# rohithr87/CILRS-Autonomous-Driving-CARLA

Hardware: AMD Instinct MI355X
Metric: frames/sec CILRS train batch=128 (higher is better)
Workload: dtype f32; 1 GPU; CILRS ResNet-34 train step (fwd+loss+bwd+Adam), Config A, 200x88 RGB, B=128/GPU, fp32; global_batch=128, parallelism=single

## Files before the change

### cilrs-autonomous-driving-carla_amd/cilrs_mi355/_lib.py

```python
from __future__ import annotations

import ctypes as C
import os

_HERE = os.path.dirname(os.path.abspath(__file__))
LIB_PATH = os.environ.get("CILRS_LIB") or os.path.join(_HERE, "libcilrs_hip.so")

c_float_p = C.POINTER(C.c_float)
vp = C.c_void_p
sz = C.c_size_t
i32 = C.c_int
i64 = C.c_int64
f32 = C.c_float
f64 = C.c_double
u64 = C.c_uint64


class Buffers(C.Structure):
    _fields_ = [("params", vp), ("grads", vp), ("bn_running", vp), ("bn_nbt", vp),
                ("workspace", vp)]


class AdamArgs(C.Structure):
    _fields_ = [("exp_avg", vp), ("exp_avg_sq", vp), ("lr", C.c_double), ("beta1", C.c_double),
# ... 134 lines not shown
    "cilrs_augment_weather_u8": (i32, [vp, vp, vp, i32, i32, i32, vp, vp, vp]),
    "cilrs_batch_assemble_weather": (i32, [vp, i64, vp, vp, vp, vp, vp, vp, i32, i32, i32, vp, vp, vp,
                                           vp, vp, vp]),
    "cilrs_augment_view_u8": (i32, [vp, vp, vp, vp, i32, i32, i32, vp, vp, vp]),
    "cilrs_batch_assemble_view": (i32, [vp, i64, vp, vp, vp, vp, vp, vp, vp, i32, i32, i32, vp, vp,
                                        vp, vp, vp, vp]),
    "cilrs_eval_acc_doubles": (i32, []),
    "cilrs_eval_accumulate": (i32, [vp, vp, vp, vp, vp, i32, vp, vp, vp]),
    "cilrs_net_profile_enable": (i32, [vp, i32]),
    "cilrs_net_profile_collect": (i32, [vp]),
    "cilrs_net_profile_count": (i32, [vp]),
    "cilrs_net_profile_entry": (i32, [vp, i32, C.c_char_p, i32, C.POINTER(C.c_longlong),
                                      C.POINTER(f64), C.POINTER(f64), C.POINTER(f64)]),
    "cilrs_net_profile_reset": (i32, [vp]),
    "cilrs_conv2d_fwd": (i32, [vp, vp, vp] + [i32] * 11 + [vp, sz, vp]),
    "cilrs_conv2d_dgrad": (i32, [vp, vp, vp, vp] + [i32] * 11 + [vp, sz, vp]),
    "cilrs_conv2d_fwd_stats": (i32, [vp, vp, vp, vp, C.POINTER(i32)] + [i32] * 10 + [vp, sz, vp]),
    "cilrs_conv2d_dgrad_bnbwd": (i32, [vp] * 7 + [i32, vp, C.POINTER(i32)] + [i32] * 10
                                 + [vp, sz, vp]),
    "cilrs_conv2d_takes_classes": (i32, [i32] * 9 + [sz, i32]),
    "cilrs_net_conv_classes": (i32, [vp, i32, C.POINTER(i32), C.POINTER(i32)]),
    "cilrs_conv2d_wgrad_scratch_floats": (sz, [i32] * 9),
    "cilrs_conv2d_wgrad": (i32, [vp, vp, vp, vp] + [i32] * 10 + [vp]),
    "cilrs_conv2d_16_scratch_halfs": (sz, [i32] * 8),
    "cilrs_conv2d_fwd_16": (i32, [vp, vp, vp, vp] + [i32] * 9 + [vp, vp]),
    "cilrs_conv2d_dgrad_16": (i32, [vp, vp, vp, vp] + [i32] * 9 + [vp, vp]),
    "cilrs_conv2d_wgrad_16_scratch_floats": (sz, [i32] * 8),
    "cilrs_conv2d_wgrad_16": (i32, [vp, vp, vp, vp] + [i32] * 9 + [vp, vp]),
    "cilrs_conv2d_train_16": (i32, [vp] * 9 + [i32, vp] + [i32] * 12 + [vp, vp]),
    "cilrs_conv2d_infer_16": (i32, [vp] * 5 + [i32] * 11 + [vp]),
    "cilrs_stem_fold_16": (i32, [vp, vp, vp, vp, i32, vp]),
    "cilrs_stem_infer_16": (i32, [vp, vp, vp, vp, i32, i32, i32, i32, vp]),
    "cilrs_maxpool_infer_16": (i32, [vp, vp, i32, i32, i32, i32, i32, vp]),
    "cilrs_avgpool_infer_16": (i32, [vp, vp, i32, i32, i32, i32, i32, vp]),
    "cilrs_bn16_train_fwd": (i32, [vp, i32, i32, vp, vp, vp, vp, vp, C.c_float, C.c_float, vp, i32,
                                   vp, vp, vp, i32, vp]),
    "cilrs_bn16_bwd": (i32, [vp, vp, vp, i32, i32, vp, vp, i32, vp, vp, vp, vp, vp, vp, i32, vp]),
    "cilrs_conv2d_wino_split": (i32, [vp, vp, vp, vp, vp, i32, i32, i32, i32, i32, vp, sz, vp, vp, vp]),
    "cilrs_conv2d_wino_scratch_floats": (sz, [i32, i32]),
    "cilrs_conv2d_wino_fwd": (i32, [vp, vp, vp, i32, i32, i32, i32, i32, vp, vp]),
    "cilrs_conv2d_wino_fold_fwd": (i32, [vp, vp, vp, vp, vp, vp, i32, i32, i32, i32, i32, i32, i32,
                                         vp, vp]),
    "cilrs_wino_filter_transform": (i32, [vp, vp, i32, i32, i32, vp]),
    "cilrs_conv2d_wino_stamps": (i32, [vp]),
    "cilrs_conv2d_wino_pre": (i32, [vp, vp, vp, vp, i32, i32, i32, i32, i32, vp]),
    "cilrs_conv2d_wino_dgrad": (i32, [vp, vp, vp, vp, i32, i32, i32, i32, i32, vp, vp]),
# ... 60 lines not shown
```

### cilrs-autonomous-driving-carla_amd/csrc/common.h

```cpp
#pragma once
#include <hip/hip_runtime.h>
#include <stdint.h>
#include <stddef.h>
#include "../../include/cilrs_hip.h"

namespace cilrs {

typedef float f32x4 __attribute__((ext_vector_type(4)));
typedef float f32x16 __attribute__((ext_vector_type(16)));

void set_error(const char* fmt, ...);
const char* last_error();

#define CILRS_CHECK(cond, ...)                   \
    do {                                         \
        if (!(cond)) {                           \
            ::cilrs::set_error(__VA_ARGS__);     \
            return 1;                            \
        }                                        \
    } while (0)

#define CILRS_HIP(expr)                                                                 \
    do {                                                                                \
        hipError_t e_ = (expr);                                                         \
// ... 108 lines not shown
    if (mode < 16) return;
    const int units = mode - 16;
    const int k = (int)((blockIdx.x >> 8) % 5u);
    for (int i = 0; i < k * units; ++i) __builtin_amdgcn_s_sleep(1);
}
#endif
int wave_priority_mode();

struct WgradArgs {
    const float* x;
    const float* dy;
    float* dw;
    float* slabs;
    int N, H, W, Cin;
    int Ho, Wo, Cout;
    int KH, KW, stride, pad;
    int x_ld, dy_ld;
    int Cin_dst;
    int accumulate;
    int prio_mode;
};
size_t wgrad_scratch_floats(const WgradArgs& a);
int launch_conv_wgrad(const WgradArgs& a, hipStream_t s);

size_t bn_partial_floats(int C);
int launch_bn_train_fwd(const float* y, int M, int C, const float* gamma, const float* beta,
                        float* running_mean, float* running_var, long long* nbt, float momentum,
                        float eps, const float* residual, int relu, float* stats, float* partial,
                        float* z, int pre_nblk, hipStream_t s, void* z16 = nullptr,
                        double* acc_head = nullptr, double* acc = nullptr);
constexpr int kBnStatsHead = 2, kBnStatsRows = 4;
int launch_bn_train_stats(const float* y, int M, int C, double* acc, float* partial, hipStream_t s);
constexpr int kMaxConvs = 56;
struct BnEvalTable {
    int n;
    int C[kMaxConvs];
    unsigned gamma[kMaxConvs], beta[kMaxConvs];
    unsigned rm[kMaxConvs], rv[kMaxConvs];
    unsigned stats[kMaxConvs];
};
int launch_bn_eval_stats_all(const BnEvalTable& t, const float* params, const float* bn_running,
                             float* ws, float eps, hipStream_t s);
struct BnStatsTable {
    int n;
    int C[kMaxConvs];
    unsigned rm[kMaxConvs], rv[kMaxConvs];
// ... 499 lines not shown
```

### cilrs-autonomous-driving-carla_amd/csrc/conv_wgrad.hip

```cpp
#include "common.h"

#include <stdlib.h>

namespace cilrs {

namespace {

constexpr int BKP = 32;

template <int BT, bool TAP_UNIFORM, bool PIN>
__global__ __launch_bounds__(256, 2) void conv_wgrad_kernel(const WgradArgs a, const int Mpix,
                                                            const int splits, const int tiles_ci,
                                                            const int Ncols, const int ntiles_x,
                                                            const int ntiles_co,
                                                            const int xcd_group) {
    constexpr int WT = BT / 2, T = WT / 32;
    constexpr int QPR = BT / 4;
    constexpr int RPP = 256 / QPR;
    constexpr int PASSES = BKP / RPP;
    constexpr int PITCH = BT + 4;

    extern __shared__ __attribute__((aligned(16))) float smem[];
    float* As = smem;
    float* Bs = smem + 2 * BKP * PITCH;

    const int tid = threadIdx.x, lane = tid & 63, wave = tid >> 6;
    const int l31 = lane & 31, lh = lane >> 5;
    const int wm = wave >> 1, wn = wave & 1;
    wave_priority(a.prio_mode < 16 ? a.prio_mode : 0);

    int logical = (int)blockIdx.x;
    if (xcd_group) {
        const int nwg = (int)gridDim.x, bid = (int)blockIdx.x;
        const int q = nwg >> 3, r = nwg & 7, xcd = bid & 7;
        const int base = xcd < r ? xcd * (q + 1) : r * (q + 1) + (xcd - r) * q;
        logical = base + (bid >> 3);
    }
    const int ntile = logical % ntiles_x;
    const int co0 = ((logical / ntiles_x) % ntiles_co) * BT;
    const int z = logical / (ntiles_x * ntiles_co);

    const int KT = (Mpix + BKP - 1) / BKP;
    const int per = (KT + splits - 1) / splits;
    const int kt_begin = z * per;
    const int kt_end = min(KT, kt_begin + per);
    const int nt = max(kt_end - kt_begin, 0);

    const int q = tid % QPR, rr = tid / QPR;

    int tap, ci, col0;
    bool col_ok;
    if constexpr (TAP_UNIFORM) {
        tap = ntile / tiles_ci;
        ci = (ntile - tap * tiles_ci) * BT + q * 4;
        col0 = tap * a.Cin + (ntile - tap * tiles_ci) * BT;
        col_ok = true;
    } else {
        col0 = ntile * BT;
        const int j = col0 + q * 4;
        tap = j / a.Cin;
        ci = j - tap * a.Cin;
        col_ok = j < Ncols;
    }
    const int kh = tap / a.KW, kw = tap - kh * a.KW;
    const int HoWo = a.Ho * a.Wo;

    const int dn = BKP / HoWo, drem = BKP - dn * HoWo;
    const int doh = drem / a.Wo, dow = drem - doh * a.Wo;
    int cn[PASSES], coh[PASSES], cow[PASSES], cp[PASSES];
#pragma unroll
    for (int i = 0; i < PASSES; ++i) {
        const int p = kt_begin * BKP + rr + RPP * i;
        cp[i] = p;
        cn[i] = p / HoWo;
        const int rem = p - cn[i] * HoWo;
        coh[i] = rem / a.Wo;
        cow[i] = rem - coh[i] * a.Wo;
    }
    const __amdgpu_buffer_rsrc_t rsDy = __builtin_amdgcn_make_buffer_rsrc(
        (void*)a.dy, 0, (int)(unsigned)((size_t)Mpix * a.dy_ld * sizeof(float)), 0x00020000);
    const __amdgpu_buffer_rsrc_t rsX = __builtin_amdgcn_make_buffer_rsrc(
        (void*)a.x, 0, (int)(unsigned)((size_t)a.N * a.H * a.W * a.x_ld * sizeof(float)),
        0x00020000);
    const unsigned dyq = (unsigned)(co0 + q * 4) * 4u;
    const unsigned dy_pitch = (unsigned)a.dy_ld * 4u;

    auto load_tile = [&](f32x4(&ra)[PASSES], f32x4(&rb)[PASSES]) {
#pragma unroll
        for (int i = 0; i < PASSES; ++i) {
            const int h = coh[i] * a.stride - a.pad + kh, w = cow[i] * a.stride - a.pad + kw;
            const bool ok = col_ok && cp[i] < Mpix && h >= 0 && w >= 0 && h < a.H && w < a.W;
            const unsigned xo =
                ok ? (unsigned)(((cn[i] * a.H + h) * a.W + w) * a.x_ld + ci) * 4u : 0xFFFFFFFFu;
            ra[i] = __builtin_bit_cast(
                f32x4, __builtin_amdgcn_raw_buffer_load_b128(
                           rsDy, (int)((unsigned)cp[i] * dy_pitch + dyq), 0, 0));
            rb[i] = __builtin_bit_cast(
                f32x4, __builtin_amdgcn_raw_buffer_load_b128(rsX, (int)xo, 0, 0));
            cp[i] += BKP;
            cow[i] += dow;
            int c1 = cow[i] >= a.Wo;
            cow[i] -= c1 ? a.Wo : 0;
            coh[i] += doh + c1;
            int c2 = coh[i] >= a.Ho;
            coh[i] -= c2 ? a.Ho : 0;
            cn[i] += dn + c2;
        }
    };
    auto store_tile = [&](int buf, const f32x4(&ra)[PASSES], const f32x4(&rb)[PASSES]) {
#pragma unroll
        for (int i = 0; i < PASSES; ++i) {
            const int row = rr + RPP * i;
            *reinterpret_cast<f32x4*>(As + (buf * BKP + row) * PITCH + q * 4) = ra[i];
            *reinterpret_cast<f32x4*>(Bs + (buf * BKP + row) * PITCH + q * 4) = rb[i];
        }
    };

    f32x16 acc[T][T];
#pragma unroll
    for (int i = 0; i < T; ++i)
#pragma unroll
        for (int j = 0; j < T; ++j)
#pragma unroll
            for (int r = 0; r < 16; ++r) acc[i][j][r] = 0.f;

    auto compute = [&](int buf) {
        if constexpr (T == 2) {
            const float* Ab = As + buf * BKP * PITCH + lh * PITCH + wm * WT + 2 * l31;
// ... 76 lines not shown
        const int col = col0 + wn * WT + 2 * l31;
#pragma unroll
        for (int i = 0; i < 2; ++i)
#pragma unroll
            for (int r = 0; r < 16; ++r) {
                const int row = (r & 3) + 8 * (r >> 2) + 4 * lh;
                const int co = co0 + wm * WT + 2 * row + i;
                float2 v;
                v.x = acc[i][0][r];
                v.y = acc[i][1][r];
                *reinterpret_cast<float2*>(out + (size_t)co * Ncols + col) = v;
            }
    } else {
        const int col = col0 + wn * WT + l31;
#pragma unroll
        for (int r = 0; r < 16; ++r) {
            const int row = (r & 3) + 8 * (r >> 2) + 4 * lh;
            const int co = co0 + wm * WT + row;
            if (col < Ncols) out[(size_t)co * Ncols + col] = acc[0][0][r];
        }
    }
}

template <int VEC>
__global__ __launch_bounds__(256) void wgrad_reduce_kernel(const float* __restrict__ slabs,
                                                           float* __restrict__ dw,
                                                           const int splits, const size_t n_src,
                                                           const int cin, const int cin_dst,
                                                           const int accumulate, const int G) {
    if constexpr (VEC == 4) {
        __shared__ f32x4 red[256];
        const int opb = 256 / G;
        const int g = threadIdx.x / opb, ol = threadIdx.x - g * opb;
        const size_t nvec = n_src / 4;
        const size_t iv = (size_t)blockIdx.x * opb + ol;
        f32x4 v = {0.f, 0.f, 0.f, 0.f};
        if (iv < nvec) {
            const float* base = slabs + iv * 4;
            f32x4 acc[4];
#pragma unroll
            for (int u = 0; u < 4; ++u) acc[u] = f32x4{0.f, 0.f, 0.f, 0.f};
            int sidx = g;
            for (; sidx + 3 * G < splits; sidx += 4 * G) {
#pragma unroll
                for (int u = 0; u < 4; ++u)
                    acc[u] += *reinterpret_cast<const f32x4*>(base + (size_t)(sidx + u * G) * n_src);
// ... 27 lines not shown
#pragma unroll
                for (int u = 0; u < 4; ++u) acc[u] += base[(size_t)(sidx + u * G) * n_src];
            }
            for (; sidx < splits; sidx += G) acc[0] += base[(size_t)sidx * n_src];
            v = (acc[0] + acc[1]) + (acc[2] + acc[3]);
        }
        if (G > 1) {
            red1[threadIdx.x] = v;
            __syncthreads();
            if (g == 0) {
                for (int k = 1; k < G; ++k) v += red1[k * opb + ol];
            }
        }
        if (g == 0 && idx < n_src) {
            const int ci = (int)(idx % cin);
            if (ci < cin_dst) {
                const size_t o = (idx / cin) * cin_dst + ci;
                dw[o] = accumulate ? dw[o] + v : v;
            }
        }
    }
}

struct WPlan { int bt; bool uniform; int tiles_ci; int ntiles; int ncols; int splits; };

double wplan_cost(double flops, int tiles, int splits, int bt, size_t out_floats) {
    static const float r128[2] = {105.f, 120.f};
    static const float r64[4] = {60.f, 85.f, 96.f, 103.f};
    const int occ = bt == 128 ? 2 : 4;
    const float* rate = bt == 128 ? r128 : r64;
    const long blocks = (long)tiles * splits;
    const long per_cu = (blocks + 255) / 256;
    const double unit = flops / (double)blocks;
    const long full = per_cu / occ, rem = per_cu % occ;
    double t = 0.0;
    if (full) t += full * unit * 256.0 * occ / (rate[occ - 1] * 1e6);
    if (rem) t += unit * 256.0 * rem / (rate[rem - 1] * 1e6);
    t += (full + (rem ? 1 : 0)) * 3.0;
    t += 4.0 + (double)out_floats * 4.0 * (2.0 * splits + 1.0) / 3.5e6;
    return t;
}

WPlan plan(const WgradArgs& a) {
    WPlan best;
    const int taps = a.KH * a.KW;
    const int Mpix = a.N * a.Ho * a.Wo;
    const int KT = cdiv(Mpix, BKP);
    const bool uniform = (a.Cin % 64) == 0;
    const size_t out_floats = (size_t)a.Cout * taps * a.Cin;
    const double flops = 2.0 * Mpix * (double)out_floats;
    static const int env_bt = experiment_env("CILRS_WGRAD_BT", 0);
    static const int env_target = experiment_env("CILRS_WGRAD_TARGET", 0);
    double bc = 1e30;
    for (int bt = 64; bt <= 128; bt += 64) {
        if (bt == 128 && !(uniform && a.Cin % 128 == 0 && a.Cout % 128 == 0)) continue;
        if (env_bt && bt != env_bt) continue;
        WPlan p;
        p.bt = bt; p.uniform = uniform; p.ncols = taps * a.Cin;
        if (uniform) { p.tiles_ci = a.Cin / bt; p.ntiles = taps * p.tiles_ci; }
        else { p.tiles_ci = 1; p.ntiles = cdiv(p.ncols, bt); }
        const int tiles = p.ntiles * (a.Cout / bt);
        const int max_splits = KT / 4 > 0 ? KT / 4 : 1;
        for (int budget = 256; budget <= 2048; budget += 256) {
            if (env_target && budget != ((env_target + 255) / 256) * 256) continue;
            int splits = budget / tiles;
            if (splits < 1) splits = 1;
            if (splits > max_splits) splits = max_splits;
            const int per = cdiv(KT, splits);
            splits = cdiv(KT, per);
            const double c = wplan_cost(flops, tiles, splits, bt, out_floats);
            if (c < bc) { bc = c; best = p; best.splits = splits; }
        }
    }
    return best;
}

}

size_t wgrad_scratch_floats(const WgradArgs& a) {
    const WPlan p = plan(a);
    return (size_t)p.splits * a.Cout * p.ncols;
}

int launch_conv_wgrad(const WgradArgs& a_in, hipStream_t s) {
    WgradArgs a = a_in;
    a.prio_mode = wave_priority_mode();
    CILRS_CHECK(a.Cout % 64 == 0, "conv_wgrad: Cout=%d must be a multiple of 64", a.Cout);
    CILRS_CHECK(a.Cin % 4 == 0 && a.x_ld % 4 == 0 && a.dy_ld % 4 == 0,
                "conv_wgrad: Cin/x_ld/dy_ld must be multiples of 4");
    CILRS_CHECK(a.slabs != nullptr, "conv_wgrad: scratch slabs missing");
    CILRS_CHECK((size_t)a.N * a.H * a.W * a.x_ld * sizeof(float) < (1ull << 32) &&
                    (size_t)a.N * a.Ho * a.Wo * a.dy_ld * sizeof(float) < (1ull << 32),
                "conv_wgrad: tensor larger than 4 GB");
    CILRS_CHECK(((uintptr_t)a.x & 15) == 0 && ((uintptr_t)a.dy & 15) == 0 &&
                    ((uintptr_t)a.slabs & 15) == 0,
                "conv_wgrad: pointers must be 16-byte aligned");
    const WPlan p = plan(a);
    const int Mpix = a.N * a.Ho * a.Wo;
    const int ntiles_co = a.Cout / p.bt;
    static const int xcd = experiment_env("CILRS_WGRAD_XCD", 1);
    dim3 grid(p.ntiles * ntiles_co * p.splits, 1, 1);
    const size_t lds = (size_t)4 * BKP * (p.bt + 4) * sizeof(float);
    static const bool pin = experiment_env("CILRS_WGRAD_PIN", 1) != 0;
    if (p.bt == 128) {
        if (set_max_dynamic_lds(reinterpret_cast<const void*>(&conv_wgrad_kernel<128, true, true>), (int)lds) ||
            set_max_dynamic_lds(reinterpret_cast<const void*>(&conv_wgrad_kernel<128, true, false>), (int)lds))
            return 1;
        if (pin)
            conv_wgrad_kernel<128, true, true><<<grid, 256, lds, s>>>(a, Mpix, p.splits,
                                                                      p.tiles_ci, p.ncols, p.ntiles, ntiles_co, xcd);
        else
            conv_wgrad_kernel<128, true, false><<<grid, 256, lds, s>>>(a, Mpix, p.splits,
                                                                       p.tiles_ci, p.ncols, p.ntiles, ntiles_co, xcd);
    } else if (p.uniform) {
        if (pin)
            conv_wgrad_kernel<64, true, true><<<grid, 256, lds, s>>>(a, Mpix, p.splits,
                                                                     p.tiles_ci, p.ncols, p.ntiles, ntiles_co, xcd);
        else
            conv_wgrad_kernel<64, true, false><<<grid, 256, lds, s>>>(a, Mpix, p.splits,
                                                                      p.tiles_ci, p.ncols, p.ntiles, ntiles_co, xcd);
    } else {
        conv_wgrad_kernel<64, false, false><<<grid, 256, lds, s>>>(a, Mpix, p.splits, p.tiles_ci,
                                                                   p.ncols, p.ntiles, ntiles_co, xcd);
    }
    CILRS_LAUNCH_CHECK();
    const size_t n_src = (size_t)a.Cout * p.ncols;
// ... 34 lines not shown
```

### cilrs-autonomous-driving-carla_amd/csrc/net.hip

```cpp
#include "common.h"
#include "../../include/cilrs_hip.h"

#include <math.h>
#include <stdarg.h>
#include <stdio.h>
#include <stdlib.h>
#include <string.h>

#include <algorithm>
#include <map>
#include <mutex>
#include <set>
#include <string>
#include <vector>

namespace cilrs {

static thread_local char g_err[1024] = "";
void set_error(const char* fmt, ...) {
    va_list ap;
    va_start(ap, fmt);
    vsnprintf(g_err, sizeof(g_err), fmt, ap);
    va_end(ap);
}
// ... 513 lines not shown
    if (bn_of && bwd_nblk) {
        a.bwd_z = ws + bn_of->z; a.bwd_y = ws + bn_of->y; a.bwd_stats = ws + bn_of->stats;
        a.bwd_relu = bn_relu; a.bwd_partial = ws + net->bn_partial; a.bwd_nblk = bwd_nblk;
        *bwd_nblk = 0;
    }
    a.N = net->B; a.H = g.H; a.W = g.W; a.Cin = c.cin;
    a.Ho = g.Ho; a.Wo = g.Wo; a.Cout = c.cout; a.K = c.k; a.stride = c.stride; a.pad = c.pad;
    a.dy_ld = c.cout; a.dx_ld = c.cin;
    a.scratch = ws + net->ksplit; a.scratch_floats = net->ksplit_floats;
    a.force_cfg = -1;
    const double flops = 2.0 * g.M * c.cout * c.k * c.k * c.cin;
    const double bytes = 4.0 * ((double)net->B * g.H * g.W * c.cin + (double)g.M * c.cout +
                                (double)c.cout * c.k * c.k * c.cin);
    RUN(net, std::string("conv_dgrad.") + kGroupName[c.group], flops, bytes, s,
        launch_conv_dgrad(a, s));
    return 0;
}

static bool wino_wgrad_on(const ConvT& c) {
    static const int env = getenv("CILRS_WINO_WGRAD") ? atoi(getenv("CILRS_WINO_WGRAD")) : 1;
    return env != 0 && wino_wgrad_supported(c.cin, c.cout, c.k, c.stride, c.pad);
}

int conv_wgrad(cilrs_net* net, const ConvT& c, const ConvG& g, const float* x, int x_cin,
               const float* dy, float* dw, float* ws, hipStream_t s) {
    if (x_cin == c.cin && !net->bf16_train && wino_wgrad_on(c)) {
        WinoWgradArgs wa;
        memset(&wa, 0, sizeof(wa));
        wa.x = x; wa.dy = dy; wa.dw = dw; wa.slabs = ws + net->slabs;
        wa.N = net->B; wa.H = g.H; wa.W = g.W; wa.C = c.cin; wa.K = c.cout;
        CILRS_CHECK(wino_wgrad_scratch_floats(net->B, g.H, g.W, c.cin, c.cout) <= net->slabs_floats,
                    "Winograd wgrad scratch too small");
        const double flops = 2.0 * g.M * c.cout * c.k * c.k * c.cin;
        const double bytes = 4.0 * ((double)net->B * g.H * g.W * c.cin + (double)g.M * c.cout +
                                    (double)c.cout * c.k * c.k * c.cin);
        RUN(net, std::string("conv_wgrad.") + kGroupName[c.group], flops, bytes, s,
            launch_conv_wino_wgrad(wa, s));
        return 0;
    }
    WgradArgs a;
    memset(&a, 0, sizeof(a));
    a.x = x; a.dy = dy; a.dw = dw; a.slabs = ws + net->slabs;
    a.N = net->B; a.H = g.H; a.W = g.W; a.Cin = x_cin;
    a.Ho = g.Ho; a.Wo = g.Wo; a.Cout = c.cout;
    a.KH = a.KW = c.k; a.stride = c.stride; a.pad = c.pad;
    a.x_ld = x_cin; a.dy_ld = c.cout; a.Cin_dst = c.cin; a.accumulate = 0;
    CILRS_CHECK(wgrad_scratch_floats(a) <= net->slabs_floats, "wgrad scratch too small");
    const double flops = 2.0 * g.M * c.cout * c.k * c.k * c.cin;
    const double bytes = 4.0 * ((double)net->B * g.H * g.W * c.cin + (double)g.M * c.cout +
// ... 227 lines not shown
        g.Ho = out_dim(height, 7, 2, 3); g.Wo = out_dim(width, 7, 2, 3);
        g.M = B * g.Ho * g.Wo;
        g.y = bump.take(trainable ? (size_t)g.M * 64 : 4);
        g.z = bump.take((size_t)g.M * 64);
        g.stats = bump.take(4 * 64);
        n->H0 = g.Ho; n->W0 = g.Wo;
        n->H1 = out_dim(g.Ho, 3, 2, 1); n->W1 = out_dim(g.Wo, 3, 2, 1);
    }
    size_t gmax = (size_t)n->cg[0].M * 64;
    size_t actmax = (size_t)B * n->H1 * n->W1 * 64;
    n->pool = bump.take((size_t)B * n->H1 * n->W1 * 64);
    const size_t argmax_floats = ((size_t)B * n->H1 * n->W1 * 64 + 3) / 4;
    n->argmax_b = bump.take(argmax_floats) * sizeof(float);
    int h = n->H1, w = n->W1;
    size_t slabs_max = 0, ksplit_max = 0;
    auto track = [&](const ConvT& c, const ConvG& g, int x_cin) {
        if (trainable) {
            WgradArgs wa;
            memset(&wa, 0, sizeof(wa));
            wa.N = B; wa.H = g.H; wa.W = g.W; wa.Cin = x_cin; wa.Ho = g.Ho; wa.Wo = g.Wo;
            wa.Cout = c.cout; wa.KH = wa.KW = c.k; wa.stride = c.stride; wa.pad = c.pad;
            const size_t sf = wgrad_scratch_floats(wa);
            if (sf > slabs_max) slabs_max = sf;
            if (x_cin == c.cin && wino_wgrad_on(c)) {
                const size_t sw = wino_wgrad_scratch_floats(B, g.H, g.W, c.cin, c.cout);
                if (sw > slabs_max) slabs_max = sw;
            }
        }
        const size_t fwd = (size_t)g.M * c.cout, bwd = (size_t)B * g.H * g.W * c.cin;
        const size_t big = fwd > bwd ? fwd : bwd;
        if (big <= (size_t)6 * 1024 * 1024 && 8 * big > ksplit_max) ksplit_max = 8 * big;
        if (fwd > actmax) actmax = fwd;
    };
    auto place = [&](int ci, int in_h, int in_w) {
        const ConvT& c = A.convs[ci];
        ConvG& g = n->cg[ci];
        g.H = in_h; g.W = in_w;
        g.Ho = out_dim(in_h, c.k, c.stride, c.pad); g.Wo = out_dim(in_w, c.k, c.stride, c.pad);
        g.M = B * g.Ho * g.Wo;
        g.y = bump.take(trainable ? (size_t)g.M * c.cout : 4);
        g.z = bump.take((size_t)g.M * c.cout);
        g.stats = bump.take(4 * c.cout);
        track(c, g, c.cin);
    };
    track(A.convs[0], n->cg[0], 4);
    for (const BlockT& blk : A.blocks) {
        place(blk.conv1, h, w);
// ... 2557 lines not shown
    memset(&a, 0, sizeof(a));
    a.x = x; a.dy = dy; a.dw = dw; a.slabs = scratch;
    a.N = N; a.H = H; a.W = W; a.Cin = Cin;
    a.Ho = (H + 2 * pad - KH) / stride + 1; a.Wo = (W + 2 * pad - KW) / stride + 1; a.Cout = Cout;
    a.KH = KH; a.KW = KW; a.stride = stride; a.pad = pad;
    a.x_ld = Cin; a.dy_ld = Cout; a.Cin_dst = Cin_dst; a.accumulate = 0;
    return a;
}

size_t cilrs_conv2d_wgrad_scratch_floats(int N, int H, int W, int Cin, int Cout, int KH, int KW,
                                         int stride, int pad) {
    return wgrad_scratch_floats(
        make_wgrad(nullptr, nullptr, nullptr, nullptr, N, H, W, Cin, Cout, KH, KW, stride, pad, Cin));
}

int cilrs_conv2d_wgrad(const float* x, const float* dy, float* dw, float* scratch, int N, int H,
                       int W, int Cin, int Cout, int KH, int KW, int stride, int pad,
                       int Cin_dst, void* stream) {
    return launch_conv_wgrad(
        make_wgrad(x, dy, dw, scratch, N, H, W, Cin, Cout, KH, KW, stride, pad, Cin_dst),
        reinterpret_cast<hipStream_t>(stream));
}

static size_t up8(size_t v) { return (v + 7) / 8 * 8; }
size_t cilrs_conv2d_16_scratch_halfs(int N, int H, int W, int Cin, int Cout, int K, int stride,
                                     int pad) {
    const int Ho = (H + 2 * pad - K) / stride + 1, Wo = (W + 2 * pad - K) / stride + 1;
    return up8((size_t)N * H * W * Cin) + up8((size_t)N * Ho * Wo * Cout) +
           2 * up8((size_t)Cout * K * K * Cin);
}

int cilrs_conv2d_fwd_16(const float* x, const float* w, float* y, float* bn_partial, int N, int H,
                        int W, int Cin, int Cout, int K, int stride, int pad, int bf16,
                        void* scratch16, void* stream) {
    CILRS_CHECK(x && w && y && scratch16, "conv2d_fwd_16: NULL argument");
    hipStream_t s = reinterpret_cast<hipStream_t>(stream);
    cilrs_half* x16 = reinterpret_cast<cilrs_half*>(scratch16);
    cilrs_half* w16 = x16 + up8((size_t)N * H * W * Cin);
    if (launch_f32_to_f16(x, x16, (size_t)N * H * W * Cin, bf16, s)) return 1;
    if (launch_f32_to_f16(w, w16, (size_t)Cout * K * K * Cin, bf16, s)) return 1;
    ConvF16Args a;
    memset(&a, 0, sizeof(a));
    a.x = x16; a.w = w16; a.y32 = y; a.bn_partial = bn_partial;
    a.N = N; a.H = H; a.W = W; a.Cin = Cin; a.Cout = Cout; a.K = K; a.stride = stride; a.pad = pad;
    a.Ho = (H + 2 * pad - K) / stride + 1; a.Wo = (W + 2 * pad - K) / stride + 1;
    a.bf16 = bf16;
// ... 316 lines not shown
```

### include/cilrs_hip.h

```cpp
#ifndef CILRS_HIP_H
#define CILRS_HIP_H

#include <stddef.h>
#include <stdint.h>

#ifdef __cplusplus
extern "C" {
#endif

typedef struct cilrs_net cilrs_net;

int cilrs_version(void);
const char* cilrs_last_error(void);

int cilrs_num_params(void);
int cilrs_num_bn(void);
size_t cilrs_param_arena_floats(void);
size_t cilrs_param_count(void);
int cilrs_param_info(int i, char* name, int name_cap, size_t* offset, size_t* numel, int* ndim,
                     int* shape4);
int cilrs_bn_info(int j, char* prefix, int prefix_cap, int* channels, size_t* rm_offset,
                  size_t* rv_offset);
size_t cilrs_bn_arena_floats(void);

// ... 354 lines not shown
                     int Cout, int KH, int KW, int stride, int pad, int force_cfg,
                     int force_splitk, float* scratch, size_t scratch_floats, void* stream);
int cilrs_conv2d_dgrad(const float* dy, const float* w, float* dx, const float* addend, int N,
                       int H, int W, int Cin, int Cout, int KH, int KW, int stride, int pad,
                       int force_cfg, int force_splitk, float* scratch, size_t scratch_floats,
                       void* stream);
int cilrs_conv2d_fwd_stats(const float* x, const float* w, float* y, float* partial, int* nblk,
                           int N, int H, int W, int Cin, int Cout, int K, int stride, int pad,
                           int force_cfg, int force_splitk, float* scratch, size_t scratch_floats,
                           void* stream);
int cilrs_conv2d_dgrad_bnbwd(const float* dy, const float* w, float* dx, const float* addend,
                             const float* bwd_z, const float* bwd_y, const float* bwd_stats,
                             int bwd_relu, float* partial, int* nblk, int N, int H, int W, int Cin,
                             int Cout, int K, int stride, int pad, int force_cfg, int force_splitk,
                             float* scratch, size_t scratch_floats, void* stream);
int cilrs_conv2d_takes_classes(int N, int H, int W, int Cin, int Cout, int K, int stride, int pad,
                               int dgrad, size_t scratch_floats, int force_splitk);
int cilrs_net_conv_classes(const cilrs_net* net, int conv, int* fwd, int* dgrad);
size_t cilrs_conv2d_wgrad_scratch_floats(int N, int H, int W, int Cin, int Cout, int KH, int KW,
                                         int stride, int pad);
int cilrs_conv2d_wgrad(const float* x, const float* dy, float* dw, float* scratch, int N, int H,
                       int W, int Cin, int Cout, int KH, int KW, int stride, int pad,
                       int Cin_dst, void* stream);

size_t cilrs_conv2d_16_scratch_halfs(int N, int H, int W, int Cin, int Cout, int K, int stride,
                                     int pad);
int cilrs_conv2d_fwd_16(const float* x, const float* w, float* y, float* bn_partial, int N, int H,
                        int W, int Cin, int Cout, int K, int stride, int pad, int bf16,
                        void* scratch16, void* stream);
int cilrs_conv2d_dgrad_16(const float* dy, const float* w, float* dx, const float* addend, int N,
                          int H, int W, int Cin, int Cout, int K, int stride, int pad, int bf16,
                          void* scratch16, void* stream);
size_t cilrs_conv2d_wgrad_16_scratch_floats(int N, int H, int W, int Cin, int Cout, int K,
                                            int stride, int pad);
int cilrs_conv2d_wgrad_16(const float* x, const float* dy, float* dw, float* scratch32, int N,
                          int H, int W, int Cin, int Cout, int K, int stride, int pad, int bf16,
                          void* scratch16, void* stream);

int cilrs_bn_bwd_frozen(const float* dz, const float* z, int M, int C, const float* gamma,
                        const float* stats, int relu, float* dy, float* g_out, void* stream);
int cilrs_bn_bwd_pool_frozen(const float* dpool, const uint8_t* argmax, const float* y, int N, int H,
                             int W, int C, const float* gamma, const float* stats, float* dy,
                             void* stream);

int cilrs_saliency_map(const float* dimage, long sn, long sc, long sh, long sw, int B, int H, int W,
                       const float* chan_scale3, float* heat, uint8_t* heat_u8, float* peak,
// ... 85 lines not shown
```

Measured before the change: 14190 frames/s.

## Add per-tap valid-rectangle wgrad kernel that skips padded pixels

Adds a weight-gradient GEMM path where each filter tap only iterates over the output-pixel rectangle whose input lies inside the image, so zero-padding contributions are neither loaded nor multiplied. Each tap gets its own split-K count from a cost model, and a dedicated reduction kernel sums a variable number of slabs per tap. It also routes small-spatial 3x3 layers away from the Winograd wgrad when the rectangle GEMM is predicted cheaper. This adds planning complexity and a per-block tap lookup, and splits are uneven across taps.

```diff
diff --git a/cilrs-autonomous-driving-carla_amd/cilrs_mi355/_lib.py b/cilrs-autonomous-driving-carla_amd/cilrs_mi355/_lib.py
--- a/cilrs-autonomous-driving-carla_amd/cilrs_mi355/_lib.py
+++ b/cilrs-autonomous-driving-carla_amd/cilrs_mi355/_lib.py
@@ -180,6 +180,8 @@
     "cilrs_net_conv_classes": (i32, [vp, i32, C.POINTER(i32), C.POINTER(i32)]),
     "cilrs_conv2d_wgrad_scratch_floats": (sz, [i32] * 9),
     "cilrs_conv2d_wgrad": (i32, [vp, vp, vp, vp] + [i32] * 10 + [vp]),
+    "cilrs_conv2d_wgrad_add": (i32, [vp, vp, vp, vp] + [i32] * 10 + [vp]),
+    "cilrs_wgrad_rect_plan": (i32, [i32] * 9 + [C.POINTER(i32)] * 3),
     "cilrs_conv2d_16_scratch_halfs": (sz, [i32] * 8),
     "cilrs_conv2d_fwd_16": (i32, [vp, vp, vp, vp] + [i32] * 9 + [vp, vp]),
     "cilrs_conv2d_dgrad_16": (i32, [vp, vp, vp, vp] + [i32] * 9 + [vp, vp]),
diff --git a/cilrs-autonomous-driving-carla_amd/csrc/common.h b/cilrs-autonomous-driving-carla_amd/csrc/common.h
--- a/cilrs-autonomous-driving-carla_amd/csrc/common.h
+++ b/cilrs-autonomous-driving-carla_amd/csrc/common.h
@@ -154,6 +154,9 @@
 };
 size_t wgrad_scratch_floats(const WgradArgs& a);
 int launch_conv_wgrad(const WgradArgs& a, hipStream_t s);
+constexpr int kWgradRectTaps = 16;
+int wgrad_rect_plan(const WgradArgs& a, int* rect, int* splits, int* smax);
+bool wgrad_rect_beats_wino(int H, int W);
 
 size_t bn_partial_floats(int C);
 int launch_bn_train_fwd(const float* y, int M, int C, const float* gamma, const float* beta,
diff --git a/cilrs-autonomous-driving-carla_amd/csrc/conv_wgrad.hip b/cilrs-autonomous-driving-carla_amd/csrc/conv_wgrad.hip
--- a/cilrs-autonomous-driving-carla_amd/csrc/conv_wgrad.hip
+++ b/cilrs-autonomous-driving-carla_amd/csrc/conv_wgrad.hip
@@ -1,6 +1,9 @@
 #include "common.h"
 
 #include <stdlib.h>
+#include <string.h>
+
+#include <type_traits>
 
 namespace cilrs {
 
@@ -8,12 +11,19 @@
 
 constexpr int BKP = 32;
 
-template <int BT, bool TAP_UNIFORM, bool PIN>
-__global__ __launch_bounds__(256, 2) void conv_wgrad_kernel(const WgradArgs a, const int Mpix,
-                                                            const int splits, const int tiles_ci,
-                                                            const int Ncols, const int ntiles_x,
-                                                            const int ntiles_co,
-                                                            const int xcd_group) {
+struct WgradRect {
+    int blk_begin[kWgradRectTaps + 1];
+    int s[kWgradRectTaps];
+    short oh0[kWgradRectTaps], ow0[kWgradRectTaps], rh[kWgradRectTaps], rw[kWgradRectTaps];
+};
+
+template <int BT, bool TAP_UNIFORM, bool PIN, bool RECT>
+__device__ __forceinline__ void conv_wgrad_body(const WgradArgs& a, const WgradRect& rc,
+                                                const int Mpix, const int splits,
+                                                const int tiles_ci, const int Ncols,
+                                                const int ntiles_x, const int ntiles_co,
+                                                const int xcd_group) {
+    static_assert(!RECT || TAP_UNIFORM, "rectangles need one tap per column tile");
     constexpr int WT = BT / 2, T = WT / 32;
     constexpr int QPR = BT / 4;
     constexpr int RPP = 256 / QPR;
@@ -36,12 +46,30 @@
         const int base = xcd < r ? xcd * (q + 1) : r * (q + 1) + (xcd - r) * q;
         logical = base + (bid >> 3);
     }
-    const int ntile = logical % ntiles_x;
-    const int co0 = ((logical / ntiles_x) % ntiles_co) * BT;
-    const int z = logical / (ntiles_x * ntiles_co);
-
-    const int KT = (Mpix + BKP - 1) / BKP;
-    const int per = (KT + splits - 1) / splits;
+    int ntile, co0, z;
+    int Kpix = Mpix, nsplit = splits;
+    int RH = a.Ho, RW = a.Wo;
+    int r_oh0 = 0, r_ow0 = 0;
+    if constexpr (RECT) {
+        int t = 0;
+#pragma unroll
+        for (int u = 1; u < kWgradRectTaps; ++u) t += logical >= rc.blk_begin[u] ? 1 : 0;
+        const int local = logical - rc.blk_begin[t];
+        ntile = t * tiles_ci + local % tiles_ci;
+        co0 = ((local / tiles_ci) % ntiles_co) * BT;
+        z = local / (tiles_ci * ntiles_co);
+        RH = rc.rh[t]; RW = rc.rw[t];
+        r_oh0 = rc.oh0[t]; r_ow0 = rc.ow0[t];
+        Kpix = a.N * RH * RW;
+        nsplit = rc.s[t];
+    } else {
+        ntile = logical % ntiles_x;
+        co0 = ((logical / ntiles_x) % ntiles_co) * BT;
+        z = logical / (ntiles_x * ntiles_co);
+    }
+
+    const int KT = (Kpix + BKP - 1) / BKP;
+    const int per = (KT + nsplit - 1) / nsplit;
     const int kt_begin = z * per;
     const int kt_end = min(KT, kt_begin + per);
     const int nt = max(kt_end - kt_begin, 0);
@@ -63,10 +91,10 @@
         col_ok = j < Ncols;
     }
     const int kh = tap / a.KW, kw = tap - kh * a.KW;
-    const int HoWo = a.Ho * a.Wo;
+    const int HoWo = RH * RW;
 
     const int dn = BKP / HoWo, drem = BKP - dn * HoWo;
-    const int doh = drem / a.Wo, dow = drem - doh * a.Wo;
+    const int doh = drem / RW, dow = drem - doh * RW;
     int cn[PASSES], coh[PASSES], cow[PASSES], cp[PASSES];
 #pragma unroll
     for (int i = 0; i < PASSES; ++i) {
@@ -74,8 +102,8 @@
         cp[i] = p;
         cn[i] = p / HoWo;
         const int rem = p - cn[i] * HoWo;
-        coh[i] = rem / a.Wo;
-        cow[i] = rem - coh[i] * a.Wo;
+        coh[i] = rem / RW;
+        cow[i] = rem - coh[i] * RW;
     }
     const __amdgpu_buffer_rsrc_t rsDy = __builtin_amdgcn_make_buffer_rsrc(
         (void*)a.dy, 0, (int)(unsigned)((size_t)Mpix * a.dy_ld * sizeof(float)), 0x00020000);
@@ -88,22 +116,33 @@
     auto load_tile = [&](f32x4(&ra)[PASSES], f32x4(&rb)[PASSES]) {
 #pragma unroll
         for (int i = 0; i < PASSES; ++i) {
-            const int h = coh[i] * a.stride - a.pad + kh, w = cow[i] * a.stride - a.pad + kw;
-            const bool ok = col_ok && cp[i] < Mpix && h >= 0 && w >= 0 && h < a.H && w < a.W;
-            const unsigned xo =
-                ok ? (unsigned)(((cn[i] * a.H + h) * a.W + w) * a.x_ld + ci) * 4u : 0xFFFFFFFFu;
+            unsigned xo, dyo;
+            if constexpr (RECT) {
+                const int oh = r_oh0 + coh[i], ow = r_ow0 + cow[i];
+                const int h = oh * a.stride - a.pad + kh, w = ow * a.stride - a.pad + kw;
+                const bool ok = cp[i] < Kpix;
+                xo = ok ? (unsigned)(((cn[i] * a.H + h) * a.W + w) * a.x_ld + ci) * 4u
+                        : 0xFFFFFFFFu;
+                dyo = ok ? (unsigned)((cn[i] * a.Ho + oh) * a.Wo + ow) * dy_pitch + dyq
+                         : 0xFFFFFFFFu;
+            } else {
+                const int h = coh[i] * a.stride - a.pad + kh, w = cow[i] * a.stride - a.pad + kw;
+                const bool ok = col_ok && cp[i] < Mpix && h >= 0 && w >= 0 && h < a.H && w < a.W;
+                xo = ok ? (unsigned)(((cn[i] * a.H + h) * a.W + w) * a.x_ld + ci) * 4u
+                        : 0xFFFFFFFFu;
+                dyo = (unsigned)cp[i] * dy_pitch + dyq;
+            }
             ra[i] = __builtin_bit_cast(
-                f32x4, __builtin_amdgcn_raw_buffer_load_b128(
-                           rsDy, (int)((unsigned)cp[i] * dy_pitch + dyq), 0, 0));
+                f32x4, __builtin_amdgcn_raw_buffer_load_b128(rsDy, (int)dyo, 0, 0));
             rb[i] = __builtin_bit_cast(
                 f32x4, __builtin_amdgcn_raw_buffer_load_b128(rsX, (int)xo, 0, 0));
             cp[i] += BKP;
             cow[i] += dow;
-            int c1 = cow[i] >= a.Wo;
-            cow[i] -= c1 ? a.Wo : 0;
+            int c1 = cow[i] >= RW;
+            cow[i] -= c1 ? RW : 0;
             coh[i] += doh + c1;
-            int c2 = coh[i] >= a.Ho;
-            coh[i] -= c2 ? a.Ho : 0;
+            int c2 = coh[i] >= RH;
+            coh[i] -= c2 ? RH : 0;
             cn[i] += dn + c2;
         }
     };
@@ -226,6 +265,27 @@
     }
 }
 
+template <int BT, bool TAP_UNIFORM, bool PIN>
+__global__ __launch_bounds__(256, 2) void conv_wgrad_kernel(const WgradArgs a, const int Mpix,
+                                                            const int splits, const int tiles_ci,
+                                                            const int Ncols, const int ntiles_x,
+                                                            const int ntiles_co,
+                                                            const int xcd_group) {
+    conv_wgrad_body<BT, TAP_UNIFORM, PIN, false>(a, WgradRect{}, Mpix, splits, tiles_ci, Ncols,
+                                                 ntiles_x, ntiles_co, xcd_group);
+}
+
+template <int BT, bool PIN>
+__global__ __launch_bounds__(256, 2) void conv_wgrad_rect_kernel(const WgradArgs a,
+                                                                 const WgradRect rc,
+                                                                 const int Mpix,
+                                                                 const int tiles_ci,
+                                                                 const int Ncols,
+                                                                 const int ntiles_co,
+                                                                 const int xcd_group) {
+    conv_wgrad_body<BT, true, PIN, true>(a, rc, Mpix, 1, tiles_ci, Ncols, 0, ntiles_co, xcd_group);
+}
+
 template <int VEC>
 __global__ __launch_bounds__(256) void wgrad_reduce_kernel(const float* __restrict__ slabs,
                                                            float* __restrict__ dw,
@@ -299,14 +359,67 @@
     }
 }
 
+template <int VEC>
+__global__ __launch_bounds__(256) void wgrad_reduce_rect_kernel(const float* __restrict__ slabs,
+                                                                float* __restrict__ dw,
+                                                                const WgradRect rc,
+                                                                const size_t n_src,
+                                                                const int ncols, const int cin,
+                                                                const int cin_dst,
+                                                                const int accumulate,
+                                                                const int G) {
+    using V = typename std::conditional<VEC == 4, f32x4, float>::type;
+    __shared__ V red[256];
+    const int opb = 256 / G;
+    const int g = threadIdx.x / opb, ol = threadIdx.x - g * opb;
+    const size_t nvec = n_src / VEC;
+    const size_t iv = (size_t)blockIdx.x * opb + ol;
+    V v = V{};
+    int splits = 0;
+    if (iv < nvec) {
+        const int tap = (int)((iv * VEC) % (size_t)ncols) / cin;
+#pragma unroll
+        for (int u = 0; u < kWgradRectTaps; ++u) splits = tap == u ? rc.s[u] : splits;
+        const float* base = slabs + iv * VEC;
+        V acc[4];
+#pragma unroll
+        for (int u = 0; u < 4; ++u) acc[u] = V{};
+        int sidx = g;
+        for (; sidx + 3 * G < splits; sidx += 4 * G) {
+#pragma unroll
+            for (int u = 0; u < 4; ++u)
+                acc[u] += *reinterpret_cast<const V*>(base + (size_t)(sidx + u * G) * n_src);
+        }
+        for (; sidx < splits; sidx += G)
+            acc[0] += *reinterpret_cast<const V*>(base + (size_t)sidx * n_src);
+        v = (acc[0] + acc[1]) + (acc[2] + acc[3]);
+    }
+    if (G > 1) {
+        red[threadIdx.x] = v;
+        __syncthreads();
+        if (g == 0) {
+            for (int k = 1; k < G; ++k) v += red[k * opb + ol];
+        }
+    }
+    if (g == 0 && iv < nvec && (splits > 0 || !accumulate)) {
+        size_t o = iv * VEC;
+        if constexpr (VEC == 1) {
+            const int ci = (int)(iv % cin);
+            if (ci >= cin_dst) return;
+            o = (iv / cin) * cin_dst + ci;
+        }
+        V* dst = reinterpret_cast<V*>(dw + o);
+        *dst = accumulate ? *dst + v : v;
+    }
+}
+
 struct WPlan { int bt; bool uniform; int tiles_ci; int ntiles; int ncols; int splits; };
 
-double wplan_cost(double flops, int tiles, int splits, int bt, size_t out_floats) {
+double wplan_gemm_cost(double flops, long blocks, int bt) {
     static const float r128[2] = {105.f, 120.f};
     static const float r64[4] = {60.f, 85.f, 96.f, 103.f};
     const int occ = bt == 128 ? 2 : 4;
     const float* rate = bt == 128 ? r128 : r64;
-    const long blocks = (long)tiles * splits;
     const long per_cu = (blocks + 255) / 256;
     const double unit = flops / (double)blocks;
     const long full = per_cu / occ, rem = per_cu % occ;
@@ -314,6 +427,11 @@
     if (full) t += full * unit * 256.0 * occ / (rate[occ - 1] * 1e6);
     if (rem) t += unit * 256.0 * rem / (rate[rem - 1] * 1e6);
     t += (full + (rem ? 1 : 0)) * 3.0;
+    return t;
+}
+
+double wplan_cost(double flops, int tiles, int splits, int bt, size_t out_floats) {
+    double t = wplan_gemm_cost(flops, (long)tiles * splits, bt);
     t += 4.0 + (double)out_floats * 4.0 * (2.0 * splits + 1.0) / 3.5e6;
     return t;
 }
@@ -352,11 +470,135 @@
     return best;
 }
 
+bool wgrad_rect_enabled() {
+    static const int env = getenv("CILRS_WGRAD_RECT") ? atoi(getenv("CILRS_WGRAD_RECT")) : 1;
+    return env != 0;
+}
+
+bool wgrad_rects(const WgradArgs& a, int* rect) {
+    auto range = [](int in, int out, int stride, int pad, int k, int* lo, int* hi) {
+        const int first = pad - k, last = in - 1 + pad - k;
+        *lo = first > 0 ? (first + stride - 1) / stride : 0;
+        *hi = last < 0 ? 0 : (last / stride + 1 < out ? last / stride + 1 : out);
+    };
+    bool smaller = false;
+    for (int kh = 0; kh < a.KH; ++kh)
+        for (int kw = 0; kw < a.KW; ++kw) {
+            int* r = rect + 4 * (kh * a.KW + kw);
+            range(a.H, a.Ho, a.stride, a.pad, kh, r + 0, r + 1);
+            range(a.W, a.Wo, a.stride, a.pad, kw, r + 2, r + 3);
+            if (r[1] <= r[0] || r[3] <= r[2]) r[0] = r[1] = r[2] = r[3] = 0;
+            if (r[1] - r[0] != a.Ho || r[3] - r[2] != a.Wo) smaller = true;
+        }
+    return smaller;
+}
+
+struct WRectPlan {
+    bool on;
+    WPlan p;
+    WgradRect rc;
+    int blocks;
+};
+
+WRectPlan plan_rect(const WgradArgs& a) {
+    WRectPlan best;
+    memset(&best, 0, sizeof(best));
+    const int taps = a.KH * a.KW;
+    if (!wgrad_rect_enabled() || (a.Cin % 64) != 0 || taps > kWgradRectTaps || a.Ho > 32767 ||
+        a.Wo > 32767)
+        return best;
+    int rect[4 * kWgradRectTaps];
+    if (!wgrad_rects(a, rect)) return best;
+    int KT[kWgradRectTaps], kt_sum = 0, kt_max = 0;
+    double pix = 0.0;
+    for (int t = 0; t < taps; ++t) {
+        const int n = a.N * (rect[4 * t + 1] - rect[4 * t]) * (rect[4 * t + 3] - rect[4 * t + 2]);
+        KT[t] = cdiv(n, BKP);
+        kt_sum += KT[t];
+        if (KT[t] > kt_max) kt_max = KT[t];
+        pix += n;
+    }
+    if (kt_sum == 0) return best;
+    const size_t tap_floats = (size_t)a.Cout * a.Cin;
+    const double flops = 2.0 * pix * (double)tap_floats;
+    static const int env_bt = experiment_env("CILRS_WGRAD_BT", 0);
+    static const int env_target = experiment_env("CILRS_WGRAD_TARGET", 0);
+    double bc = 1e30;
+    for (int bt = 64; bt <= 128; bt += 64) {
+        if (bt == 128 && !(a.Cin % 128 == 0 && a.Cout % 128 == 0)) continue;
+        if (env_bt && bt != env_bt) continue;
+        const int tiles_ci = a.Cin / bt;
+        const int tiles = tiles_ci * (a.Cout / bt);
+        for (int budget = 256; budget <= 2048; budget += 256) {
+            if (env_target && budget != ((env_target + 255) / 256) * 256) continue;
+            const int slabs_fit = budget / tiles > 0 ? budget / tiles : 1;
+            int L = cdiv(kt_sum, slabs_fit);
+            if (L < 4) L = 4;
+            if (L > kt_max) L = kt_max;
+            int s[kWgradRectTaps], ssum = 0, smax = 0;
+            for (;; ++L) {
+                ssum = smax = 0;
+                for (int t = 0; t < taps; ++t) {
+                    s[t] = KT[t] ? cdiv(KT[t], L) : 0;
+                    if (s[t]) s[t] = cdiv(KT[t], cdiv(KT[t], s[t]));
+                    ssum += s[t];
+                    if (s[t] > smax) smax = s[t];
+                }
+                if (ssum <= slabs_fit || L >= kt_max) break;
+            }
+            double c = wplan_gemm_cost(flops, (long)tiles * ssum, bt);
+            c += 4.0 + 4.0 * ((double)tap_floats * (2.0 * ssum + taps)) / 3.5e6;
+            if (c < bc) {
+                bc = c;
+                best.on = true;
+                best.p.bt = bt; best.p.uniform = true; best.p.tiles_ci = tiles_ci;
+                best.p.ntiles = taps * tiles_ci; best.p.ncols = taps * a.Cin;
+                best.p.splits = smax;
+                best.blocks = tiles * ssum;
+                int begin = 0;
+                for (int t = 0; t < kWgradRectTaps; ++t) {
+                    best.rc.blk_begin[t] = begin;
+                    best.rc.s[t] = t < taps ? s[t] : 0;
+                    begin += best.rc.s[t] * tiles;
+                    best.rc.oh0[t] = t < taps ? (short)rect[4 * t] : 0;
+                    best.rc.rh[t] = t < taps ? (short)(rect[4 * t + 1] - rect[4 * t]) : 0;
+                    best.rc.ow0[t] = t < taps ? (short)rect[4 * t + 2] : 0;
+                    best.rc.rw[t] = t < taps ? (short)(rect[4 * t + 3] - rect[4 * t + 2]) : 0;
+                }
+                best.rc.blk_begin[kWgradRectTaps] = begin;
+            }
+        }
+    }
+    return best;
+}
+
 }
 
 size_t wgrad_scratch_floats(const WgradArgs& a) {
-    const WPlan p = plan(a);
+    const WRectPlan r = plan_rect(a);
+    const WPlan p = r.on ? r.p : plan(a);
     return (size_t)p.splits * a.Cout * p.ncols;
+}
+
+int wgrad_rect_plan(const WgradArgs& a, int* rect, int* splits, int* smax) {
+    const int taps = a.KH * a.KW;
+    if (a.N < 1 || a.H < 1 || a.W < 1 || a.Ho < 1 || a.Wo < 1 || a.KH < 1 || a.KW < 1 ||
+        a.stride < 1 || a.pad < 0 || taps > kWgradRectTaps || a.Cin < 1 || a.Cout < 1)
+        return -1;
+    wgrad_rects(a, rect);
+    const WRectPlan r = plan_rect(a);
+    const int plain = r.on ? 0 : plan(a).splits;
+    for (int t = 0; t < taps; ++t) splits[t] = r.on ? r.rc.s[t] : plain;
+    *smax = r.on ? r.p.splits : plain;
+    return r.on ? 1 : 0;
+}
+
+bool wgrad_rect_beats_wino(int H, int W) {
+    if (!wgrad_rect_enabled()) return false;
+    constexpr double kRate = 1.25;
+    const double wino = 16.0 * ((H + 1) / 2) * ((W + 1) / 2);
+    const int rows = (H > 1 ? 2 * (H - 1) : 0) + H, cols = (W > 1 ? 2 * (W - 1) : 0) + W;
+    return (double)rows * cols < kRate * wino;
 }
 
 int launch_conv_wgrad(const WgradArgs& a_in, hipStream_t s) {
@@ -372,13 +614,49 @@
     CILRS_CHECK(((uintptr_t)a.x & 15) == 0 && ((uintptr_t)a.dy & 15) == 0 &&
                     ((uintptr_t)a.slabs & 15) == 0,
                 "conv_wgrad: pointers must be 16-byte aligned");
-    const WPlan p = plan(a);
+    const WRectPlan rp = plan_rect(a);
+    const WPlan p = rp.on ? rp.p : plan(a);
     const int Mpix = a.N * a.Ho * a.Wo;
     const int ntiles_co = a.Cout / p.bt;
     static const int xcd = experiment_env("CILRS_WGRAD_XCD", 1);
-    dim3 grid(p.ntiles * ntiles_co * p.splits, 1, 1);
+    dim3 grid(rp.on ? rp.blocks : p.ntiles * ntiles_co * p.splits, 1, 1);
     const size_t lds = (size_t)4 * BKP * (p.bt + 4) * sizeof(float);
     static const bool pin = experiment_env("CILRS_WGRAD_PIN", 1) != 0;
+    if (rp.on) {
+        if (p.bt == 128) {
+            if (set_max_dynamic_lds(reinterpret_cast<const void*>(&conv_wgrad_rect_kernel<128, true>), (int)lds) ||
+                set_max_dynamic_lds(reinterpret_cast<const void*>(&conv_wgrad_rect_kernel<128, false>), (int)lds))
+                return 1;
+            if (pin)
+                conv_wgrad_rect_kernel<128, true><<<grid, 256, lds, s>>>(a, rp.rc, Mpix, p.tiles_ci,
+                                                                         p.ncols, ntiles_co, xcd);
+            else
+                conv_wgrad_rect_kernel<128, false><<<grid, 256, lds, s>>>(a, rp.rc, Mpix, p.tiles_ci,
+                                                                          p.ncols, ntiles_co, xcd);
+        } else if (pin) {
+            conv_wgrad_rect_kernel<64, true><<<grid, 256, lds, s>>>(a, rp.rc, Mpix, p.tiles_ci,
+                                                                    p.ncols, ntiles_co, xcd);
+        } else {
+            conv_wgrad_rect_kernel<64, false><<<grid, 256, lds, s>>>(a, rp.rc, Mpix, p.tiles_ci,
+                                                                     p.ncols, ntiles_co, xcd);
+        }
+        CILRS_LAUNCH_CHECK();
+        const size_t n_src = (size_t)a.Cout * p.ncols;
+        const bool vec = a.Cin == a.Cin_dst && ((uintptr_t)a.dw & 15) == 0;
+        const size_t nout = vec ? n_src / 4 : n_src;
+        int G = 1;
+        while (G < 16 && nout * G < (vec ? 131072u : 262144u) && 8 * G <= p.splits) G *= 2;
+        const int opb = 256 / G;
+        const int nblk = (int)((nout + opb - 1) / opb);
+        if (vec)
+            wgrad_reduce_rect_kernel<4><<<nblk, 256, 0, s>>>(a.slabs, a.dw, rp.rc, n_src, p.ncols,
+                                                             a.Cin, a.Cin_dst, a.accumulate, G);
+        else
+            wgrad_reduce_rect_kernel<1><<<nblk, 256, 0, s>>>(a.slabs, a.dw, rp.rc, n_src, p.ncols,
+                                                             a.Cin, a.Cin_dst, a.accumulate, G);
+        CILRS_LAUNCH_CHECK();
+        return 0;
+    }
     if (p.bt == 128) {
         if (set_max_dynamic_lds(reinterpret_cast<const void*>(&conv_wgrad_kernel<128, true, true>), (int)lds) ||
             set_max_dynamic_lds(reinterpret_cast<const void*>(&conv_wgrad_kernel<128, true, false>), (int)lds))
diff --git a/cilrs-autonomous-driving-carla_amd/csrc/net.hip b/cilrs-autonomous-driving-carla_amd/csrc/net.hip
--- a/cilrs-autonomous-driving-carla_amd/csrc/net.hip
+++ b/cilrs-autonomous-driving-carla_amd/csrc/net.hip
@@ -559,9 +559,13 @@
     return env != 0 && wino_wgrad_supported(c.cin, c.cout, c.k, c.stride, c.pad);
 }
 
+static bool wino_wgrad_takes(const ConvT& c, const ConvG& g) {
+    return wino_wgrad_on(c) && !wgrad_rect_beats_wino(g.H, g.W);
+}
+
 int conv_wgrad(cilrs_net* net, const ConvT& c, const ConvG& g, const float* x, int x_cin,
                const float* dy, float* dw, float* ws, hipStream_t s) {
-    if (x_cin == c.cin && !net->bf16_train && wino_wgrad_on(c)) {
+    if (x_cin == c.cin && !net->bf16_train && wino_wgrad_takes(c, g)) {
         WinoWgradArgs wa;
         memset(&wa, 0, sizeof(wa));
         wa.x = x; wa.dy = dy; wa.dw = dw; wa.slabs = ws + net->slabs;
@@ -835,7 +839,7 @@
             wa.Cout = c.cout; wa.KH = wa.KW = c.k; wa.stride = c.stride; wa.pad = c.pad;
             const size_t sf = wgrad_scratch_floats(wa);
             if (sf > slabs_max) slabs_max = sf;
-            if (x_cin == c.cin && wino_wgrad_on(c)) {
+            if (x_cin == c.cin && wino_wgrad_takes(c, g)) {
                 const size_t sw = wino_wgrad_scratch_floats(B, g.H, g.W, c.cin, c.cout);
                 if (sw > slabs_max) slabs_max = sw;
             }
@@ -3439,6 +3443,24 @@
         reinterpret_cast<hipStream_t>(stream));
 }
 
+int cilrs_conv2d_wgrad_add(const float* x, const float* dy, float* dw, float* scratch, int N, int H,
+                           int W, int Cin, int Cout, int KH, int KW, int stride, int pad,
+                           int Cin_dst, void* stream) {
+    WgradArgs a = make_wgrad(x, dy, dw, scratch, N, H, W, Cin, Cout, KH, KW, stride, pad, Cin_dst);
+    a.accumulate = 1;
+    return launch_conv_wgrad(a, reinterpret_cast<hipStream_t>(stream));
+}
+
+int cilrs_wgrad_rect_plan(int N, int H, int W, int Cin, int Cout, int KH, int KW, int stride,
+                          int pad, int* rect, int* splits, int* smax) {
+    if (!rect || !splits || !smax || KH < 1 || KW < 1 || stride < 1 || pad < 0 ||
+        H + 2 * pad < KH || W + 2 * pad < KW)
+        return -1;
+    return wgrad_rect_plan(
+        make_wgrad(nullptr, nullptr, nullptr, nullptr, N, H, W, Cin, Cout, KH, KW, stride, pad, Cin),
+        rect, splits, smax);
+}
+
 static size_t up8(size_t v) { return (v + 7) / 8 * 8; }
 size_t cilrs_conv2d_16_scratch_halfs(int N, int H, int W, int Cin, int Cout, int K, int stride,
                                      int pad) {
diff --git a/include/cilrs_hip.h b/include/cilrs_hip.h
--- a/include/cilrs_hip.h
+++ b/include/cilrs_hip.h
@@ -400,6 +400,11 @@
 int cilrs_conv2d_wgrad(const float* x, const float* dy, float* dw, float* scratch, int N, int H,
                        int W, int Cin, int Cout, int KH, int KW, int stride, int pad,
                        int Cin_dst, void* stream);
+int cilrs_conv2d_wgrad_add(const float* x, const float* dy, float* dw, float* scratch, int N, int H,
+                           int W, int Cin, int Cout, int KH, int KW, int stride, int pad,
+                           int Cin_dst, void* stream);
+int cilrs_wgrad_rect_plan(int N, int H, int W, int Cin, int Cout, int KH, int KW, int stride,
+                          int pad, int* rect, int* splits, int* smax);
 
 size_t cilrs_conv2d_16_scratch_halfs(int N, int H, int W, int Cin, int Cout, int K, int stride,
                                      int pad);
```

Result: no change. 14310 frames/s (median of 6 runs) (+0.8%).
